# atonderski/future-object-detection

Hardware: AMD Instinct MI355X
Metric: frame-sequences/sec fwd+bwd, T=6 900x1600 (higher is better)
Workload: dtype bf16; 1 GPU; spatiotemporal ConditionalDETR (ResNet-50, 6 enc + 6 dec layers, 128 queries), T=6 frames 900x1600, batch 2/GPU, num_images K=5 (5 past frames live), random-init weights; step = forward (incl. Hungarian set loss, post-proc, AP bookkeeping) + backward + clip + AdamW; global_batch=2, frames=6, num_images=5, parallelism=dp1

## Files before the change

### future-object-detection_amd/csrc/api.cpp

```cpp
#include <stdarg.h>
#include <stdio.h>
#include <stdlib.h>
#include <string.h>

#include <mutex>

#include "../../include/fod.h"
#include "knobs.h"

static thread_local char g_err[512] = "";

void fod_set_error(const char* fmt, ...) {
  va_list ap;
  va_start(ap, fmt);
  vsnprintf(g_err, sizeof(g_err), fmt, ap);
  va_end(ap);
}

extern "C" size_t fod_last_error(char* buf, size_t cap) {
  const size_t n = strlen(g_err);
  if (buf && cap) {
    const size_t c = n < cap - 1 ? n : cap - 1;
    memcpy(buf, g_err, c);
    buf[c] = 0;
  }
  return n;
}

extern "C" int fod_abi_version(void) { return FOD_ABI_VERSION; }

extern "C" size_t fod_workspace_bytes(int kind) {
  switch (kind) {
    case FOD_WS_NT_SPLIT: return (size_t)FOD_NT_SPLIT_WS_FLOATS * sizeof(float);
    case FOD_WS_NT_SPLIT_TICKETS: return (size_t)FOD_NT_SPLIT_TICKETS * sizeof(unsigned);
    case FOD_WS_TN_PARTIALS: return FOD_TN_WS_BYTES;
    case FOD_WS_ATTN_SPLIT_PER_TILE: return (size_t)FOD_ATTN_SPLIT_WS_FLOATS_PER_TILE * sizeof(float);
    case FOD_WS_DET: return FOD_DET_WS_BYTES;
    case FOD_WS_TN_MULTI_DET: return FOD_TN_MULTI_DET_WS_BYTES;
    default: return 0;
  }
}

namespace {
struct KnobName {
  const char* name;
  int Knobs::*i;
  double Knobs::*d;
};
const KnobName KNOB_NAMES[] = {
    {"FOD_NT_SMALL", &Knobs::nt_small, nullptr},
    {"FOD_NT_NARROW", &Knobs::nt_narrow, nullptr},
    {"FOD_NT_SPLITK", &Knobs::nt_splitk, nullptr},
    {"FOD_NT_BIG", &Knobs::nt_big, nullptr},
    {"FOD_NT_BIG256", &Knobs::nt_big256, nullptr},
    {"FOD_NT_BIG_ILV", &Knobs::nt_big_ilv, nullptr},
    {"FOD_NT_BIG256_MINK", &Knobs::nt_big256_mink, nullptr},
    {"FOD_NT_BIG_MINK", &Knobs::nt_big_mink, nullptr},
    {"FOD_NT_BIG_MINN", &Knobs::nt_big_minn, nullptr},
    {"FOD_TN_SMALL", &Knobs::tn_small, nullptr},
    {"FOD_TN_BIG", &Knobs::tn_big, nullptr},
    {"FOD_TN_BIG_DENSE", &Knobs::tn_big_dense, nullptr},
    {"FOD_TN_BIG256", &Knobs::tn_big256, nullptr},
    {"FOD_TN_BIG_MIN", nullptr, &Knobs::tn_big_min},
    {"FOD_TN_BIG_SPLITS", &Knobs::tn_big_splits, nullptr},
    {"FOD_TN_WS", &Knobs::tn_ws, nullptr},
    {"FOD_TN_XCD", &Knobs::tn_xcd, nullptr},
    {"FOD_TN_ROWS", &Knobs::tn_rows, nullptr},
    {"FOD_ATTN_LDS", &Knobs::attn_lds, nullptr},
    {"FOD_ATTN_PF", &Knobs::attn_pf, nullptr},
    {"FOD_FP8_STAGE", &Knobs::fp8_stage, nullptr},
    {"FOD_LN_BWD_GROUPS", &Knobs::ln_bwd_groups, nullptr},
    {"FOD_BNK_VERSION", &Knobs::bnk_version, nullptr},
};

bool knob_parse(const KnobName& k, const char* text, Knobs& t) {
  char* end = nullptr;
  if (k.d) {
    const double v = strtod(text, &end);
    if (end == text || *end) return false;
    t.*k.d = v;
    return true;
  }
  if (Knobs{}.*k.i == Knobs::AUTO && !strcmp(text, "auto")) {
    t.*k.i = Knobs::AUTO;
    return true;
  }
  const long v = strtol(text, &end, 10);
  if (end == text || *end || v < 0 || v > 0x7FFFFFFF) return false;
  t.*k.i = (int)v;
  return true;
}

std::mutex g_knob_mutex;
Knobs& knob_table() {
  static Knobs table = [] {
    Knobs t;
    for (const KnobName& k : KNOB_NAMES)
      if (const char* text = getenv(k.name)) knob_parse(k, text, t);
    return t;
  }();
  return table;
}
const KnobName* knob_find(const char* name) {
  for (const KnobName& k : KNOB_NAMES)
    if (name && !strcmp(name, k.name)) return &k;
// ... 43 lines not shown
```

### future-object-detection_amd/csrc/common.h

```cpp
#pragma once
#include <hip/hip_runtime.h>
#include <stdint.h>

#include <mutex>

#include "../../include/fod.h"

typedef __attribute__((ext_vector_type(8))) __bf16 bf16x8_t;
typedef __attribute__((ext_vector_type(4))) __bf16 bf16x4_t;
typedef __attribute__((ext_vector_type(16))) float f32x16;
typedef __attribute__((ext_vector_type(4))) float f32x4;
typedef __attribute__((ext_vector_type(4))) short short4_t;

#define FOD_DEVINL __device__ __forceinline__

void fod_set_error(const char* fmt, ...);
#define FOD_REQUIRE(cond, ...)          \
  do {                                  \
    if (!(cond)) {                      \
      fod_set_error(__VA_ARGS__);       \
      return FOD_ERR_ARG;               \
    }                                   \
  } while (0)
#define FOD_LAUNCH_CHECK()                                              \
// ... 64 lines not shown
  for (int j = 0; j < 8; ++j) acc = __builtin_amdgcn_mfma_f32_32x32x2f32(a.v[j], b.v[j], acc, 0, 0, 0);
}

FOD_DEVINL void frag_load_contig(Frag<__bf16>& f, const __bf16* p) {
  f.v = *reinterpret_cast<const bf16x8_t*>(p);
}
FOD_DEVINL void frag_load_contig(Frag<float>& f, const float* p) {
  const f32x4 a = *reinterpret_cast<const f32x4*>(p);
  const f32x4 b = *reinterpret_cast<const f32x4*>(p + 4);
  f.v[0] = a[0]; f.v[1] = a[1]; f.v[2] = a[2]; f.v[3] = a[3];
  f.v[4] = b[0]; f.v[5] = b[1]; f.v[6] = b[2]; f.v[7] = b[3];
}
template <typename T>
FOD_DEVINL void frag_zero(Frag<T>& f) {
#pragma unroll
  for (int j = 0; j < 8; ++j) f.v[j] = (T)0.f;
}
template <typename T>
FOD_DEVINL void frag_from_acc(Frag<T>& f, const f32x16& acc, int s) {
#pragma unroll
  for (int j = 0; j < 8; ++j) f.v[j] = (T)acc[8 * s + j];
}
template <typename T>
FOD_DEVINL void frag_gather_accorder(Frag<T>& f, const T* base, long stride, int s, int h, int nrows) {
#pragma unroll
  for (int j = 0; j < 8; ++j) {
    const int r = 16 * s + 8 * (j >> 2) + 4 * h + (j & 3);
    f.v[j] = (r < nrows) ? base[(long)r * stride] : (T)0.f;
  }
}

FOD_DEVINL unsigned drop_mix(unsigned i, unsigned seed_lo, unsigned seed_hi) {
  unsigned h = (i ^ seed_lo) * 0x9E3779B1u + seed_hi;
  h ^= h >> 15;
  h *= 0x85EBCA77u;
  h ^= h >> 13;
  h *= 0xC2B2AE3Du;
  h ^= h >> 16;
  return h;
}

FOD_DEVINL unsigned long long mix64(unsigned long long x) {
  x = (x ^ (x >> 30)) * 0xBF58476D1CE4E5B9ull;
  x = (x ^ (x >> 27)) * 0x94D049BB133111EBull;
  return x ^ (x >> 31);
}
FOD_DEVINL unsigned long long effective_seed(unsigned long long seed, const unsigned long long* base_dev) {
  return base_dev ? mix64(seed + *base_dev) : seed;
}

FOD_DEVINL void store_sc1(float* p, float v) { __hip_atomic_store(p, v, __ATOMIC_RELAXED, __HIP_MEMORY_SCOPE_AGENT); }
FOD_DEVINL float load_sc1(const float* p) { return __hip_atomic_load(p, __ATOMIC_RELAXED, __HIP_MEMORY_SCOPE_AGENT); }
FOD_DEVINL void stores_done() { asm volatile("s_waitcnt vmcnt(0)" ::: "memory"); }

FOD_DEVINL int acc_row(int reg, int lane) { return (reg & 3) + 8 * (reg >> 2) + 4 * (lane >> 5); }

FOD_DEVINL float wave_sum(float v) {
#pragma unroll
  for (int o = 32; o > 0; o >>= 1) v += __shfl_xor(v, o);
  return v;
}
FOD_DEVINL float wave_max(float v) {
#pragma unroll
  for (int o = 32; o > 0; o >>= 1) v = fmaxf(v, __shfl_xor(v, o));
  return v;
}

static inline int ceil_div(long a, long b) { return (int)((a + b - 1) / b); }

struct LdsLimitOnce {
  std::once_flag once[64];
  int rc[64];
};
static inline int fod_lds_limit_once(LdsLimitOnce& st, const void* kernel, size_t bytes, const char* who) {
  int dev = 0;
  if (hipGetDevice(&dev) != hipSuccess || dev < 0 || dev >= 64) {
    fod_set_error("%s: no current device", who);
    return FOD_ERR_RUNTIME;
  }
  std::call_once(st.once[dev], [&] {
    st.rc[dev] = hipFuncSetAttribute(kernel, hipFuncAttributeMaxDynamicSharedMemorySize, (int)bytes) == hipSuccess ? 0 : 1;
  });
  if (st.rc[dev]) {
    fod_set_error("%s: cannot raise the dynamic LDS limit to %zu", who, bytes);
    return FOD_ERR_RUNTIME;
  }
  return FOD_OK;
}
```

### future-object-detection_amd/csrc/gemm_nt.hip

```cpp
#include <stdlib.h>

#include <type_traits>

#include "common.h"
#include "gemm_nt.h"
#include "gemm_tn.h"

namespace {

using namespace fodnt;

template <typename T, int MODE, int NT, bool UTAP>
FOD_DEVINL void gemm_nt_body(const NtParams& p) {
  constexpr int VEC = Elem<T>::VEC;
  constexpr int BK = ROW_BYTES / (int)sizeof(T);
  constexpr int BN = 64 * NT;
  constexpr int KSTEPS = BK / 16;
  constexpr int BROWS = BN / 32;
  extern __shared__ __attribute__((aligned(16))) unsigned char smem[];
  unsigned char* sA = smem;
  unsigned char* sB = smem + 2 * BM * ROW_BYTES;

  const int tid = threadIdx.x;
  const int lane = tid & 63;
  const int wave = tid >> 6;
  const int wm = wave >> 1, wn = wave & 1;
  FOD_STAMP(0);
  const int xcd = blockIdx.x & 7, slot = blockIdx.x >> 3;
  const int nt_i = slot % p.gx;
  const int mt_i = (slot / p.gx) * 8 + xcd;
  if (mt_i >= p.gy) return;
  const int n0 = nt_i * BN;
  const int m0 = mt_i * BM;
  const int cc = tid & 7;
  const int r0 = tid >> 3;

  constexpr unsigned OOB = 0xFFFFFFF0u;
  const auto rsA = __builtin_amdgcn_make_buffer_rsrc(const_cast<void*>(p.A), 0, p.a_bytes, 0x00020000);
  const auto rsB = __builtin_amdgcn_make_buffer_rsrc(const_cast<void*>(p.B), 0, p.b_bytes, 0x00020000);

  unsigned a_base[4];
  int a_h[4], a_w[4];
  int px_img = 0, px_h = 0, px_w = 0;
  if (MODE != MODE_DENSE) {
    const int mfirst = m0 + r0;
    const int hw = p.Hd * p.Wd;
    px_img = mfirst / hw;
    const int rem = mfirst - px_img * hw;
    px_h = rem / p.Wd;
    px_w = rem - px_h * p.Wd;
  }
#pragma unroll
  for (int i = 0; i < 4; ++i) {
    const int m = m0 + r0 + 32 * i;
    const bool valid = m < p.M;
    if (MODE == MODE_DENSE) {
      const int row = p.a_row_mod > 0 ? (m % p.a_row_mod) : m;
// ... 484 lines not shown
#pragma unroll
    for (int j = 0; j < 2; ++j)
#pragma unroll
      for (int r = 0; r < 16; ++r) acc[i][j][r] = 0.f;
  auto compute = [&](const Unit& f) {
#pragma unroll
    for (int ks = 0; ks < 2; ++ks)
#pragma unroll
      for (int i = 0; i < 2; ++i)
#pragma unroll
        for (int j = 0; j < 2; ++j) mma16(f.a[ks][i], f.b[ks][j], acc[i][j]);
  };
  Unit f0, f1;
  load_unit(ub, f0);
  load_unit(ub + 1, f1);
  FOD_STAMP(1);
  for (int u = ub; u < ue; u += 2) {
    compute(f0);
    load_unit(u + 2, f0);
    if (u + 1 < ue) compute(f1);
    load_unit(u + 3, f1);
  }

  FOD_STAMP(2);
#pragma unroll
  for (int i = 0; i < 2; ++i)
#pragma unroll
    for (int j = 0; j < 2; ++j)
#pragma unroll
      for (int r = 0; r < 16; ++r) sC[wave][i * 32 + acc_row(r, lane)][j * 32 + fr] = acc[i][j][r];
  __syncthreads();
  FOD_STAMP(3);
  const bool has_scale = p.scale != nullptr, has_mask = p.mask != nullptr;
  long c_base = bz * p.c_batch;
  int n_c = n;
  if (p.c_seg_cols > 0) {
    const int cseg = n0 / p.c_seg_cols;
    c_base += (long)cseg * p.c_seg_stride;
    n_c = n - cseg * p.c_seg_cols;
  }
  f32x4 vsum[4];
#pragma unroll
  for (int ps = 0; ps < 4; ++ps) {
    const int row = rq + 16 * ps;
    vsum[ps] = *reinterpret_cast<const f32x4*>(&sC[0][row][cq * 4]);
#pragma unroll
    for (int w = 1; w < 4; ++w) vsum[ps] += *reinterpret_cast<const f32x4*>(&sC[w][row][cq * 4]);
  }
  if (KS > 1) {
    __shared__ unsigned s_ticket;
    const long tile = (long)blockIdx.y * gridDim.x + blockIdx.x;
    float* mine = p.split_ws + (tile * KS + kz) * 4096;
#pragma unroll
    for (int ps = 0; ps < 4; ++ps)
#pragma unroll
      for (int e = 0; e < 4; ++e) store_sc1(mine + (rq + 16 * ps) * 64 + cq * 4 + e, vsum[ps][e]);
    stores_done();
    __syncthreads();
    if (tid == 0) s_ticket = atomicAdd(p.split_tickets + tile, 1u);
    __syncthreads();
    if (s_ticket != (unsigned)(KS - 1)) return;
    const float* all = p.split_ws + tile * KS * 4096;
#pragma unroll
    for (int ps = 0; ps < 4; ++ps) vsum[ps] = f32x4{0.f, 0.f, 0.f, 0.f};
    for (int z = 0; z < KS; ++z)
#pragma unroll
      for (int ps = 0; ps < 4; ++ps)
#pragma unroll
        for (int e = 0; e < 4; ++e) vsum[ps][e] += load_sc1(all + z * 4096 + (rq + 16 * ps) * 64 + cq * 4 + e);
    if (tid == 0) p.split_tickets[tile] = 0u;
  }
#pragma unroll
  for (int ps = 0; ps < 4; ++ps) {
    const int row = rq + 16 * ps;
    const int m = m0 + row;
    f32x4 v = vsum[ps];
    if (has_scale) v = v * sc;
    v += sh;
#pragma unroll
    for (int e = 0; e < 4; ++e) v[e] += (float)rres[ps][e];
    if (p.relu) {
#pragma unroll
      for (int e = 0; e < 4; ++e) v[e] = fmaxf(v[e], 0.f);
    }
    if (has_mask) {
#pragma unroll
      for (int e = 0; e < 4; ++e) v[e] = ((float)rmsk[ps][e] > 0.f) ? v[e] : 0.f;
    }
    if (m < p.M && n_ok) {
      if (p.c_is_f32) {
        *reinterpret_cast<f32x4*>(reinterpret_cast<float*>(p.C) + c_base + (long)m * p.ldc + n_c) = v;
      } else {
        *reinterpret_cast<bf16x4_t*>(reinterpret_cast<__bf16*>(p.C) + c_base + (long)m * p.ldc + n_c) =
            bf16x4_t{(__bf16)v[0], (__bf16)v[1], (__bf16)v[2], (__bf16)v[3]};
      }
    }
  }
  FOD_STAMP(4);
}

template <typename T, int MODE>
int launch_128(const NtParams& p, const NtRoute& r, hipStream_t stream) {
  NtParams q = p;
  q.gy = ceil_div(p.M, BM);
  const bool narrow = r.tile_n == 64;
  const dim3 block(256);
  constexpr int BK = ROW_BYTES / (int)sizeof(T);
  const bool utap = MODE != MODE_DENSE && MODE != MODE_STEM && p.Cs % BK == 0;
  q.gx = ceil_div(p.N, r.tile_n);
  const dim3 grid(q.gx * ((q.gy + 7) / 8 * 8));
  const size_t lds = 2 * (BM + r.tile_n) * ROW_BYTES;
#define FOD_NT_LAUNCH(KERNEL_NT1, KERNEL_NT2)                                        \
  do {                                                                               \
    if (narrow) hipLaunchKernelGGL((KERNEL_NT1), grid, block, lds, stream, q);       \
    else hipLaunchKernelGGL((KERNEL_NT2), grid, block, lds, stream, q);              \
  } while (0)
  if constexpr (MODE == MODE_DENSE) {
    FOD_NT_LAUNCH((gemm_nt_kernel<T, 1>), (gemm_nt_kernel<T, 2>));
  } else if constexpr (MODE == MODE_STEM) {
    FOD_NT_LAUNCH((conv_stem_fwd_kernel<T, 1>), (conv_stem_fwd_kernel<T, 2>));
  } else if constexpr (MODE == MODE_CONV) {
    if (utap) FOD_NT_LAUNCH((conv2d_fwd_kernel<T, 1, true>), (conv2d_fwd_kernel<T, 2, true>));
// ... 160 lines not shown
  FOD_REQUIRE(out && (dtype == FOD_BF16 || dtype == FOD_F32), "gemm_nt_route: bad args");
  NtParams p{};
  if (int rc = dense_params(p, dtype, nullptr, lda, a_row_mod, nullptr, ldb, nullptr, ldc, M, N, K, epi)) return rc;
  *out = route(MODE_DENSE, dtype, p, fod_knobs());
  return FOD_OK;
}

extern "C" int fod_gemm_nt_grouped(int dtype, const void* A, long lda, int a_seg_len, long a_seg_stride,
                                   const void* B, long ldb, void* C, long ldc, int c_seg_cols, long c_seg_stride,
                                   int M, int N, int K, const fod_epilogue* epi, int res_nseg, long res_seg_stride,
                                   hipStream_t stream) {
  FOD_REQUIRE(dtype == FOD_BF16, "gemm_nt_grouped: bf16 only (dtype %d)", dtype);
  FOD_REQUIRE(A && B && C, "gemm_nt_grouped: null operand");
  FOD_REQUIRE(M > 0 && N > 0 && K > 0, "gemm_nt_grouped: empty problem %d %d %d", M, N, K);
  FOD_REQUIRE(K % 8 == 0 && lda % 8 == 0 && ldb % 8 == 0, "gemm_nt_grouped: K=%d lda=%ld ldb=%ld must be multiples of 8",
              K, lda, ldb);
  FOD_REQUIRE(((uintptr_t)A % 16) == 0 && ((uintptr_t)B % 16) == 0, "gemm_nt_grouped: operands must be 16-byte aligned");
  FOD_REQUIRE(a_seg_len >= 0 && c_seg_cols >= 0, "gemm_nt_grouped: negative segment size");
  FOD_REQUIRE(a_seg_len == 0 || (a_seg_len % 32 == 0 && K % a_seg_len == 0 && a_seg_stride % 8 == 0),
              "gemm_nt_grouped: A segments of %d (stride %ld) must be multiples of 32 dividing K=%d", a_seg_len,
              a_seg_stride, K);
  FOD_REQUIRE(c_seg_cols == 0 || (c_seg_cols % 64 == 0 && c_seg_stride % 4 == 0),
              "gemm_nt_grouped: C segments of %d columns (stride %ld) must be multiples of 64 / 4", c_seg_cols,
              c_seg_stride);
  NtParams p{};
  p.A = A; p.B = B; p.C = C;
  p.lda = lda; p.ldb = ldb; p.ldc = ldc;
  p.M = M; p.N = N; p.K = K;
  p.a_seg_len = a_seg_len; p.a_seg_stride = a_seg_stride;
  p.c_seg_cols = c_seg_cols; p.c_seg_stride = c_seg_stride;
  fill_epilogue(p, epi);
  decide_vec_epilogue(p);
  FOD_REQUIRE(p.vec_epi, "gemm_nt_grouped: N, ldc and the epilogue operands must be 4-element / 16-byte aligned");
  FOD_REQUIRE(res_nseg >= 0 && (res_nseg == 0 || (p.res && c_seg_cols > 0 && res_seg_stride % 4 == 0 &&
                                                  res_nseg <= ceil_div(N, c_seg_cols))),
              "gemm_nt_grouped: per-segment residual (%d blocks) needs a residual, C segments and a 4-element block stride", res_nseg);
  p.res_nseg = res_nseg;
  p.res_seg_stride = res_seg_stride;
  FOD_REQUIRE(!p.res || ((long)(res_nseg > 1 ? res_nseg - 1 : 0) * res_seg_stride +
                         (long)(p.res_row_mod > 0 ? p.res_row_mod : M) * p.ldr + N) * 2 < 0x7FFFFFF0L,
              "gemm_nt_grouped: residual larger than 2 GiB");
  FOD_REQUIRE(!p.mask || ((long)M * p.ldmask + N) * 2 < 0x7FFFFFF0L, "gemm_nt_grouped: mask larger than 2 GiB");
  const long nseg = a_seg_len > 0 ? K / a_seg_len : 1;
  const long seg_k = a_seg_len > 0 ? a_seg_len : K;
  const long ab = ((nseg - 1) * a_seg_stride + (long)(M - 1) * lda + seg_k) * 2, bb = ((long)(N - 1) * ldb + K) * 2;
  FOD_REQUIRE(ab < 0xFFFFFFF0L - 16 && bb < 0xFFFFFFF0L - 16, "gemm_nt_grouped: operand larger than 4 GiB");
  p.a_bytes = (unsigned)ab;
  p.b_bytes = (unsigned)bb;
  hipLaunchKernelGGL(gemm_nt_small_kernel, dim3(ceil_div(N, 64), ceil_div(M, 64)), dim3(256), 0, stream, p);
  FOD_LAUNCH_CHECK();
  return FOD_OK;
}

extern "C" int fod_gemm_nt_batched(int dtype, int batches, const void* A, long lda, long a_batch, const void* B, long ldb,
                                   long b_batch, void* C, long ldc, long c_batch, int M, int N, int K,
                                   const fod_epilogue* epi, long shift_batch, long residual_batch, long mask_batch,
                                   hipStream_t stream) {
  FOD_REQUIRE(dtype == FOD_BF16, "gemm_nt_batched: bf16 only (dtype %d)", dtype);
  FOD_REQUIRE(A && B && C && batches > 0, "gemm_nt_batched: null operand / no batch");
  FOD_REQUIRE(M > 0 && N > 0 && K > 0, "gemm_nt_batched: empty problem %d %d %d", M, N, K);
  FOD_REQUIRE(K % 8 == 0 && lda % 8 == 0 && ldb % 8 == 0, "gemm_nt_batched: K=%d lda=%ld ldb=%ld must be multiples of 8",
              K, lda, ldb);
  FOD_REQUIRE(a_batch % 8 == 0 && b_batch % 8 == 0 && c_batch % 8 == 0 && shift_batch % 4 == 0 && residual_batch % 8 == 0 &&
                  mask_batch % 8 == 0,
              "gemm_nt_batched: batch strides must keep every operand 16-byte aligned");
  FOD_REQUIRE(((uintptr_t)A % 16) == 0 && ((uintptr_t)B % 16) == 0, "gemm_nt_batched: operands must be 16-byte aligned");
  NtParams p{};
  p.A = A; p.B = B; p.C = C;
  p.lda = lda; p.ldb = ldb; p.ldc = ldc;
  p.M = M; p.N = N; p.K = K;
  fill_epilogue(p, epi);
  p.split_ws = nullptr; p.split_tickets = nullptr;
  decide_vec_epilogue(p);
  FOD_REQUIRE(p.vec_epi, "gemm_nt_batched: N, ldc and the epilogue operands must be 4-element / 16-byte aligned");
  FOD_REQUIRE(!p.res || p.res_row_mod == 0, "gemm_nt_batched: no periodic residual");
  FOD_REQUIRE(!p.res || ((long)M * p.ldr + N) * 2 < 0x7FFFFFF0L, "gemm_nt_batched: residual larger than 2 GiB");
  FOD_REQUIRE(!p.mask || ((long)M * p.ldmask + N) * 2 < 0x7FFFFFF0L, "gemm_nt_batched: mask larger than 2 GiB");
  const long ab = ((long)(M - 1) * lda + K) * 2, bb = ((long)(N - 1) * ldb + K) * 2;
  FOD_REQUIRE(ab < 0xFFFFFFF0L - 16 && bb < 0xFFFFFFF0L - 16, "gemm_nt_batched: operand larger than 4 GiB");
  p.a_bytes = (unsigned)ab;
  p.b_bytes = (unsigned)bb;
  const long gy = (long)ceil_div(M, 64) * batches;
  FOD_REQUIRE(gy <= 65535, "gemm_nt_batched: %ld row tiles x batches exceed the grid", gy);
  p.batches = batches;
  p.a_batch = a_batch; p.b_batch = b_batch; p.c_batch = c_batch;
  p.shift_batch = shift_batch; p.res_batch = residual_batch; p.mask_batch = mask_batch;
  hipLaunchKernelGGL(gemm_nt_small_kernel, dim3(ceil_div(N, 64), (unsigned)gy), dim3(256), 0, stream, p);
  FOD_LAUNCH_CHECK();
  return FOD_OK;
}

namespace {
int conv_params(NtParams& p, int dtype, bool dgrad, const void* src, const void* w, void* dst, const fod_conv_geom* g,
                const fod_epilogue* epi) {
  const int vec = dtype == FOD_BF16 ? 8 : 4;
  FOD_REQUIRE(g->stride == 1 || g->stride == 2, "conv: stride %d unsupported", g->stride);
  const int Ho = (g->H + 2 * g->pad - g->kh) / g->stride + 1;
  const int Wo = (g->W + 2 * g->pad - g->kw) / g->stride + 1;
  FOD_REQUIRE(Ho == g->Ho && Wo == g->Wo, "conv: geometry mismatch Ho=%d/%d Wo=%d/%d", g->Ho, Ho, g->Wo, Wo);
  FOD_REQUIRE(g->Cin % vec == 0 && g->Cout % vec == 0, "conv: channels %d/%d must be multiples of %d",
              g->Cin, g->Cout, vec);
  FOD_REQUIRE(((uintptr_t)src % 16) == 0 && ((uintptr_t)w % 16) == 0, "conv: operands must be 16-byte aligned");
  p.A = src; p.B = w; p.C = dst;
  p.kh = g->kh; p.kw = g->kw; p.stride = g->stride; p.pad = g->pad;
  if (!dgrad) {
    p.Hs = g->H; p.Ws = g->W; p.Cs = g->Cin;
// ... 125 lines not shown
```

### future-object-detection_amd/csrc/knobs.h

```cpp
#pragma once

struct Knobs {
  static constexpr int AUTO = -1;
  int nt_small = 1;
  int nt_narrow = AUTO;
  int nt_splitk = AUTO;
  int nt_big = 1;
  int nt_big256 = 1;
  int nt_big_ilv = AUTO;
  int nt_big256_mink = 128;
  int nt_big_mink = 1536;
  int nt_big_minn = 256;
  int tn_small = 1;
  int tn_big = 1;
  int tn_big_dense = 0;
  int tn_big256 = 0;
  double tn_big_min = 2.0e9;
  int tn_big_splits = 0;
  int tn_ws = 1;
  int tn_xcd = 1;
  int tn_rows = 0;
  int attn_lds = 8;
  int attn_pf = 1;
  int fp8_stage = 1;
  int ln_bwd_groups = 4;
  int bnk_version = 4;
};

Knobs fod_knobs();
```

### future-object-detection_amd/future_od/native/lib.py

```python
import contextlib
import ctypes as C
import os

from . import abi
from .abi import FodError
from ..switches import SW

LIB_PATH = os.path.normpath(os.path.join(os.path.dirname(os.path.abspath(__file__)), "..", "..", "lib", "libfod_hip.so"))

globals().update({name[4:].replace("ROUTE_", "", 1): value for name, value in abi.CONSTANTS.items()})

_i, _l, _f, _p = C.c_int, C.c_long, C.c_float, C.c_void_p


def _struct(name, c_name):
    return type(name, (C.Structure,), {"_fields_": [(field, abi.CTYPE[kind]) for field, kind in abi.STRUCTS[c_name]]})


Epilogue = _struct("Epilogue", "fod_epilogue")
ConvGeom = _struct("ConvGeom", "fod_conv_geom")
AttnShape = _struct("AttnShape", "fod_attn_shape")
PermuteJob = _struct("PermuteJob", "fod_permute_job")
TnJob = _struct("TnJob", "fod_tn_job")
NtRoute = _struct("NtRoute", "fod_nt_route")
TnRoute = _struct("TnRoute", "fod_tn_route")
AttnRoute = _struct("AttnRoute", "fod_attn_kernels")

EXPORTS = sorted(abi.PROTOTYPES)
SIGNATURES = {name: [abi.CTYPE[kind] for kind in args] for name, args in abi.served(abi.PROTOTYPES).items()}
EXT_EXPORTS = sorted(abi.EXT_PROTOTYPES)
EXT_SIGNATURES = {name: [abi.CTYPE[kind] for kind in args] for name, args in abi.served(abi.EXT_PROTOTYPES).items()}


def _typed(lib, name):
    ret, args = abi.PROTOTYPES[name] if name in abi.PROTOTYPES else abi.EXT_PROTOTYPES[name]
    fn = getattr(lib, name)
    fn.restype, fn.argtypes = abi.CTYPE[ret], [abi.CTYPE[kind] for kind in args]
    return fn


def _load():
    if not os.path.isfile(LIB_PATH):
        raise FodError(
            f"{LIB_PATH} not found: build it with `python -c 'import __graft_entry__ as g; g.build()'` "
            "(or future-object-detection_amd/build.sh). There is no fallback path.")
    import torch
    lib = C.CDLL(LIB_PATH)
    built = _typed(lib, "fod_abi_version")()
    if built != abi.CONSTANTS["FOD_ABI_VERSION"]:
        raise FodError(f"libfod_hip.so ABI {built} != header ABI {abi.CONSTANTS['FOD_ABI_VERSION']}: rebuild")
    for name in EXPORTS + EXT_EXPORTS:
        if not hasattr(lib, name):
            raise FodError(f"libfod_hip.so does not export {name}: rebuild")
        _typed(lib, name)
    return lib


LIB = _load()


def last_error():
    buf = C.create_string_buffer(512)
    LIB.fod_last_error(buf, 512)
    return buf.value.decode("utf-8", "replace")


def knob(name):
    buf = C.create_string_buffer(32)
    if LIB.fod_knob_get(name.encode(), buf, 32) != 0:
        raise FodError(f"fod_knob_get failed: {last_error()}")
    return buf.value.decode()


def set_knob(name, value):
    if LIB.fod_knob_set(name.encode(), None if value is None else str(value).encode()) != 0:
        raise FodError(f"fod_knob_set failed: {last_error()}")


@contextlib.contextmanager
def knobs(**values):
    old = {name: knob(name) for name in values}
    try:
        for name, value in values.items():
            set_knob(name, value)
        yield
    finally:
        for name, value in old.items():
            set_knob(name, value)


def _load_fast():
    import importlib.util
    path = os.path.join(os.path.dirname(LIB_PATH), "_fodfast.so")
    if not os.path.isfile(path) or not SW.FOD_FASTCALL:
        return {}
    spec = importlib.util.spec_from_file_location("_fodfast", path)
    mod = importlib.util.module_from_spec(spec)
    spec.loader.exec_module(mod)
    return {name: getattr(mod, name) for name in SIGNATURES if hasattr(mod, name)}


FAST = _load_fast()
_ENTRY = {name: FAST.get(name, getattr(LIB, name)) for name in SIGNATURES}
_ENTRY.update({name: getattr(LIB, name) for name in EXT_SIGNATURES})


def _plain_call(name, *args):
    rc = _ENTRY[name](*args)
    if rc != 0:
        raise FodError(f"{name} failed ({rc}): {last_error()}")


class Profiler:

    def __init__(self):
        self.enabled = False
        self.records = []
        self.pending_work = 0.0

    def start(self):
        self.enabled = True
        self.records = []

    def stop(self):
        self.enabled = False

    def summary(self):
# ... 29 lines not shown
```

### future-object-detection_amd/future_od/native/ops.py

```python
import ctypes as C
import math

import torch

from . import abi, capture
from . import lib as L
from .lib import F32, BF16, AttnShape, ConvGeom, Epilogue
from .. import switches
from ..switches import SW


def call(name, *args, **kw):
    return L.call(name, *args, **kw)

_DT = {torch.float32: F32, torch.bfloat16: BF16}


def dt(t):
    try:
        return _DT[t.dtype]
    except KeyError:
        raise L.FodError(f"unsupported activation dtype {t.dtype}") from None


# ... 7 lines not shown


class _Addr(int):

    def __new__(cls, struct):
        self = super().__new__(cls, C.addressof(struct))
        self.keep = struct
        return self


def ptr(t):
    if t is None:
        return None
    return t.data_ptr()


def _chk(t, name, dtype=None):
    if not t.is_cuda:
        raise L.FodError(f"{name}: expected a device tensor (the HIP path has no CPU fallback)")
    if not t.is_contiguous():
        raise L.FodError(f"{name}: expected a contiguous tensor, got strides {t.stride()} for {tuple(t.shape)}")
    if dtype is not None and t.dtype != dtype:
        raise L.FodError(f"{name}: expected {dtype}, got {t.dtype}")
    return t


_WS = {}


def _workspace(kind, device, captured=None):
    if captured is None:
        captured = torch.cuda.is_current_stream_capturing()
    key = (kind, device.index, "graph" if captured else stream())
    hit = _WS.get(key)
    if hit is None:
        nbytes = L.LIB.fod_workspace_bytes(kind)
        hit = torch.zeros(nbytes // 4, dtype=torch.int32, device=device)
        _WS[key] = hit
    if captured:
        capture.hold_or_ask("scratch", hit)
    return hit


def preallocate_graph_workspaces(device):
    device = torch.device(device)
    kinds = (L.WS_NT_SPLIT, L.WS_NT_SPLIT_TICKETS, L.WS_TN_PARTIALS)
    if SW.FOD_DETERMINISTIC:
        kinds += (L.WS_DET, L.WS_TN_MULTI_DET)
    for kind in kinds:
        _workspace(kind, device, captured=True)
    tiles = max((hit[2] for key, hit in _ATTN_SPLIT.items() if key[0] == device.index), default=0)
    if tiles:
        _attn_split_workspace(device, tiles, captured=True)


def set_deterministic(flag):
    switches.set("FOD_DETERMINISTIC", bool(flag))


def is_deterministic():
    return SW.FOD_DETERMINISTIC


def det_workspace(device, kind=L.WS_DET):
    ws = _workspace(kind, device)
    return ws.data_ptr(), ws.numel() * 4


_DET_TWINS = abi.det_twins(abi.PROTOTYPES)


def call_twin(name, device, *args, **kw):
    if not SW.FOD_DETERMINISTIC:
        return call(name, *args, stream(), **kw)
    scratch = det_workspace(device) if _DET_TWINS[name] else ()
    return call(name + "_det", *args, *scratch, stream(), **kw)


def nt_wants_split_ws(M, N, K):
    return K >= 1024 and ((M + 63) // 64) * ((N + 63) // 64) <= 64


def tn_may_use_partials_ws(M):
    return M >= 8192


def _epi(scale=None, shift=None, residual=None, ld_residual=0, residual_row_mod=0, relu_mask=None,
         ld_mask=0, relu=False, out_f32=False, split_for=None):
    want_split = split_for is not None and nt_wants_split_ws(*split_for[1:])
    if (scale is None and shift is None and residual is None and relu_mask is None and not relu and not out_f32
            and not want_split):
        return None
    ws = tk = None
    if want_split:
        ws, tk = _workspace(L.WS_NT_SPLIT, split_for[0]), _workspace(L.WS_NT_SPLIT_TICKETS, split_for[0])
    e = Epilogue(ptr(scale), ptr(shift), ptr(residual), ld_residual, residual_row_mod,
                 ptr(relu_mask), ld_mask, int(relu), int(out_f32), ptr(ws), ptr(tk))
    return _Addr(e)


def tn_workspace(device):
    ws = _workspace(L.WS_TN_PARTIALS, device)
    return ws.data_ptr(), ws.numel() * 4


_THERE = 16


def gemm_nt_route(M, N, K, dtype=torch.bfloat16):
    e, r = Epilogue(), L.NtRoute()
    if dtype == torch.bfloat16 and nt_wants_split_ws(M, N, K):
        e.split_ws = e.split_tickets = _THERE
    call("fod_gemm_nt_route", _DT[dtype], K, 0, K, N, M, N, K, C.addressof(e), C.addressof(r))
    return r


def _tn_ws_bytes(M):
    return L.LIB.fod_workspace_bytes(L.WS_TN_PARTIALS) if tn_may_use_partials_ws(M) or SW.FOD_DETERMINISTIC else 0


def gemm_tn_route(M, N1, K2, dtype=torch.bfloat16, row_scale=False, colsum=False):
    r = L.TnRoute()
    call("fod_gemm_tn_route", _DT[dtype], M, N1, K2, N1, K2, K2, int(row_scale), int(colsum), int(SW.FOD_DETERMINISTIC),
         _tn_ws_bytes(M), C.addressof(r))
    return r


def conv2d_route(which, geom, dtype=torch.bfloat16):
    r = L.TnRoute() if which == L.CONV_WGRAD else L.NtRoute()
    call("fod_conv2d_route", which, _DT[dtype], C.addressof(geom), None, int(SW.FOD_DETERMINISTIC),
         _tn_ws_bytes(geom.Nimg * geom.Ho * geom.Wo), C.addressof(r))
    return r


def gemm_nt(a, b, *, a_row_mod=0, m_rows=None, scale=None, shift=None, residual=None,
            residual_row_mod=0, relu=False, relu_mask=None, out_f32=False, out=None):
    _chk(a, "a"); _chk(b, "b", a.dtype)
    K = a.shape[-1]
    N = b.shape[0]
    assert b.shape[1] == K, (a.shape, b.shape)
    a_rows = a.numel() // K
    M = m_rows if m_rows is not None else a_rows
    if a_row_mod:
        assert a_row_mod <= a_rows
    else:
        assert M <= a_rows
    for v, n in ((scale, "scale"), (shift, "shift")):
        if v is not None:
            _chk(v, n, torch.float32); assert v.numel() == N
    if residual is not None:
        _chk(residual, "residual", a.dtype)
        assert residual.shape[-1] == N
        rr = residual.numel() // N
        assert (residual_row_mod and residual_row_mod <= rr) or (not residual_row_mod and rr >= M)
    if relu_mask is not None:
        _chk(relu_mask, "relu_mask", a.dtype)
        assert relu_mask.numel() == M * N
    if out is None:
        out = torch.empty((M, N), dtype=torch.float32 if out_f32 else a.dtype, device=a.device)
    else:
        _chk(out, "out"); assert out.numel() == M * N
    call("fod_gemm_nt", dt(a), ptr(a), K, a_row_mod, ptr(b), K, ptr(out), N, M, N, K,
         _epi(scale, shift, residual, N, residual_row_mod, relu_mask, N, relu, out_f32,
              split_for=(a.device, M, N, K) if a.dtype == torch.bfloat16 else None), stream(),
         work=2.0 * M * N * K)
    return out


def gemm_nt_batched(a, b, *, b_cols=False, shift=None, residual=None, relu=False, relu_mask=None):
    _chk(a, "a", torch.bfloat16); _chk(b, "b", torch.bfloat16)
    P, M, K = a.shape
    if b_cols:
        N = b.shape[0]
        assert b.dim() == 2 and b.shape[1] == P * K, (a.shape, b.shape)
        ldb, b_batch = P * K, K
    else:
        N = b.numel() // (P * K)
        assert b.shape[-1] == K and N * P * K == b.numel(), (a.shape, b.shape)
        ldb, b_batch = K, N * K
    if shift is not None:
        _chk(shift, "shift", torch.float32); assert shift.numel() == P * N
    for v, n in ((residual, "residual"), (relu_mask, "relu_mask")):
        if v is not None:
            _chk(v, n, torch.bfloat16); assert v.numel() == P * M * N
    out = torch.empty((P, M, N), dtype=a.dtype, device=a.device)
    call("fod_gemm_nt_batched", dt(a), P, ptr(a), K, M * K, ptr(b), ldb, b_batch, ptr(out), N, M * N, M, N, K,
         _epi(None, shift, residual, N, 0, relu_mask, N, relu, False), N, M * N, M * N, stream(),
         work=2.0 * P * M * N * K, tag="fod_gemm_nt")
    return out


def gemm_tn_acc(g, x, dw, row_scale=None, colsum=None, zeroed=False):
    _chk(g, "g"); _chk(x, "x", g.dtype); _chk(dw, "dw", torch.float32)
    N1, K2 = g.shape[-1], x.shape[-1]
    M = g.numel() // N1
    assert x.numel() // K2 == M and dw.numel() == N1 * K2, (g.shape, x.shape, dw.shape)
    if row_scale is not None:
        _chk(row_scale, "row_scale", torch.float32); assert row_scale.numel() == N1
    if colsum is not None:
        _chk(colsum, "colsum", torch.float32); assert colsum.numel() == N1
    ws, ws_bytes = tn_workspace(g.device) if _tn_ws_bytes(M) else (None, 0)
    call_twin("fod_gemm_tn_acc", g.device, dt(g), ptr(g), N1, ptr(x), K2, ptr(dw), K2, M, N1, K2, ptr(row_scale),
              ptr(colsum), 0 if zeroed else 1, ws, ws_bytes, work=2.0 * M * N1 * K2, tag="fod_gemm_tn_acc")
    return dw


def group_linear_fwd(x, wcat, bcat, P, relu=False, residual=None, res_row_mod=0):
    _chk(x, "x", torch.bfloat16); _chk(wcat, "wcat", torch.bfloat16)
    K = x.shape[-1]
    rows = x.numel() // K
    N = wcat.shape[0]
    D = N // P
    assert wcat.shape[1] == K and N == P * D and D % 64 == 0, (x.shape, wcat.shape, P)
    if bcat is not None:
        _chk(bcat, "bcat", torch.float32); assert bcat.numel() == N
    y = torch.empty((P, rows, D), dtype=x.dtype, device=x.device)
    nseg, seg_stride = 0, 0
    if residual is not None:
        _chk(residual, "residual", x.dtype)
        nseg, R = residual.shape[0], residual.shape[1]
        assert residual.dim() == 3 and residual.shape[2] == D and nseg <= P
        assert (res_row_mod and res_row_mod <= R) or (not res_row_mod and R >= rows)
        seg_stride = R * D
    call("fod_gemm_nt_grouped", dt(x), ptr(x), K, 0, 0, ptr(wcat), K, ptr(y), D, D, rows * D, rows, N, K,
         _epi(None, bcat, residual, D, res_row_mod, None, N, relu, False), nseg, seg_stride, stream(),
         work=2.0 * rows * N * K, tag="fod_gemm_nt")
    return y


def group_linear_dgrad(g, wcat_t, P):
    _chk(g, "g", torch.bfloat16); _chk(wcat_t, "wcat_t", torch.bfloat16)
    _, rows, D = g.shape
    K = wcat_t.shape[0]
    assert g.shape[0] == P and wcat_t.shape[1] == P * D and D % 32 == 0
    dx = torch.empty((rows, K), dtype=g.dtype, device=g.device)
    call("fod_gemm_nt_grouped", dt(g), ptr(g), D, D, rows * D, ptr(wcat_t), P * D, ptr(dx), K, 0, 0, rows, K, P * D,
         None, 0, 0, stream(), work=2.0 * rows * K * P * D, tag="fod_gemm_nt")
    return dx


def group_linear_wgrad(g, x, dw, db, zeroed=False):
    _chk(g, "g", torch.bfloat16); _chk(x, "x", torch.bfloat16); _chk(dw, "dw", torch.float32)
    P, rows, D = g.shape
    K = x.shape[-1]
    assert x.numel() // K == rows and dw.numel() == P * D * K and D % 64 == 0
    if db is not None:
        _chk(db, "db", torch.float32); assert db.numel() == P * D
    call("fod_gemm_tn_grouped", dt(g), ptr(g), D, D, rows * D, ptr(x), K, ptr(dw), K, rows, P * D, K, ptr(db),
         0 if zeroed else 1, stream(), work=2.0 * rows * P * D * K, tag="fod_gemm_tn_acc")
    return dw


def colsum_acc(g, out, group_rows=0):
    _chk(g, "g"); _chk(out, "out", torch.float32)
    N = g.shape[-1]
    M = g.numel() // N
    groups = 1 if group_rows <= 0 else (M + group_rows - 1) // group_rows
    assert out.numel() == groups * N, (g.shape, out.shape, group_rows)
    call_twin("fod_colsum_acc", g.device, dt(g), ptr(g), N, M, N, group_rows, ptr(out))
    return out


def conv_geom(x_shape, cout, k, stride, pad):
    n, h, w, cin = x_shape
    ho = (h + 2 * pad - k) // stride + 1
    wo = (w + 2 * pad - k) // stride + 1
    return ConvGeom(n, h, w, cin, ho, wo, cout, k, k, stride, pad)


def _conv_flops(g, cin=None):
    return 2.0 * g.Nimg * g.Ho * g.Wo * g.Cout * g.kh * g.kw * (g.Cin if cin is None else cin)


def conv2d_fwd(x, w, geom, *, scale=None, shift=None, residual=None, relu=False, work_cin=None, out=None):
    _chk(x, "x"); _chk(w, "w", x.dtype)
    assert tuple(x.shape) == (geom.Nimg, geom.H, geom.W, geom.Cin), (x.shape, geom.H, geom.W, geom.Cin)
    assert w.numel() == geom.Cout * geom.kh * geom.kw * geom.Cin
    if out is None:
        y = torch.empty((geom.Nimg, geom.Ho, geom.Wo, geom.Cout), dtype=x.dtype, device=x.device)
    else:
        y = _chk(out, "out", x.dtype)
        assert tuple(y.shape) == (geom.Nimg, geom.Ho, geom.Wo, geom.Cout), (y.shape,)
    for v in (scale, shift):
        if v is not None:
            _chk(v, "scale/shift", torch.float32); assert v.numel() == geom.Cout
    if residual is not None:
        _chk(residual, "residual", x.dtype); assert residual.shape == y.shape
    call("fod_conv2d_fwd", dt(x), ptr(x), ptr(w), ptr(y), _Addr(geom),
# ... 770 lines not shown
```

### include/fod.h

```cpp
#ifndef FOD_H_
#define FOD_H_

#include <stddef.h>
#include <stdint.h>

#ifdef __cplusplus
extern "C" {
#endif

typedef struct ihipStream_t* fod_stream_t;

enum { FOD_F32 = 0, FOD_BF16 = 1 };
enum { FOD_OK = 0, FOD_ERR_ARG = 1, FOD_ERR_LAUNCH = 2, FOD_ERR_RUNTIME = 3 };

size_t fod_last_error(char* buf, size_t cap);
int fod_abi_version(void);
#define FOD_ABI_VERSION 12

int fod_knob_set(const char* name, const char* value);
int fod_knob_get(const char* name, char* out, size_t out_bytes);

enum { FOD_ROUTE_NT_SMALL = 0,
       FOD_ROUTE_NT_128 = 1,
       FOD_ROUTE_NT_BIG = 2 };
typedef struct fod_nt_route {
  int kernel;
  int tile_n;
  int stages;
  int interleave;
  int ksplit;
  int wants_split_ws;
} fod_nt_route;
enum { FOD_ROUTE_TN_SMALL = 0,
       FOD_ROUTE_TN_128 = 1,
       FOD_ROUTE_TN_BIG = 2 };
typedef struct fod_tn_route {
  int kernel;
  int bi, bj;
  int nsplit;
  int m_per_split;
  int xcd_order;
  int uses_partials_ws;
} fod_tn_route;

typedef struct fod_epilogue {
  const float* scale;
  const float* shift;
  const void* residual;
  long ld_residual;
  int residual_row_mod;
  const void* relu_mask;
  long ld_mask;
  int relu;
  int out_f32;
  void* split_ws;
  void* split_tickets;
} fod_epilogue;
#define FOD_NT_SPLIT_WS_FLOATS (64 * 8 * 4096)
#define FOD_NT_SPLIT_TICKETS 64
#define FOD_TN_WS_BYTES ((size_t)64 << 20)
enum { FOD_WS_NT_SPLIT = 0, FOD_WS_NT_SPLIT_TICKETS = 1, FOD_WS_TN_PARTIALS = 2, FOD_WS_ATTN_SPLIT_PER_TILE = 3,
       FOD_WS_DET = 4, FOD_WS_TN_MULTI_DET = 5 };
size_t fod_workspace_bytes(int kind);
#define FOD_DET_WS_BYTES ((size_t)16 << 20)
#define FOD_TN_MULTI_DET_WS_BYTES ((size_t)128 << 20)
#define FOD_TN_DET_MAX_SPLITS 4

int fod_gemm_nt(int dtype, const void* A, long lda, int a_row_mod, const void* B, long ldb, void* C,
                long ldc, int M, int N, int K, const fod_epilogue* epi, fod_stream_t stream);

// ... 293 lines not shown
```

### include/fod_ext.h

```cpp
#ifndef FOD_EXT_H_
#define FOD_EXT_H_

#include "fod.h"

#ifdef __cplusplus
extern "C" {
#endif

int fod_multi_ema(const long* pairs, const long* numel, const int* blk_tensor, const int* blk_chunk, int nblocks,
                  const long long* updates_dev, float decay, int warmup, fod_stream_t stream);
int fod_multi_swap(const long* pairs, const long* numel, const int* blk_tensor, const int* blk_chunk, int nblocks,
                   fod_stream_t stream);
int fod_multi_accum(const long* pairs, const long* numel, const int* blk_tensor, const int* blk_chunk, int nblocks,
                    int mode, float scale, fod_stream_t stream);
int fod_clip_crop_resize_photo(const unsigned char* src, float* dst, int B, int L, int C, int H0, int W0, int H, int W,
                               long src_stride_b, long src_stride_l, const int* plans, const float* mean,
                               const float* std, const float* photo, fod_stream_t stream);

#ifdef __cplusplus
}
#endif
#endif
```

Baseline: 108.9 frame-sequences/s.

## Add split-K deep GEMM path for small-tile, long-K NT GEMMs and grouped dgrad

Adds a new entry point that launches the small NT GEMM kernel with a split-K grid chosen by a planner. It applies when the output has few 64x64 tiles but a long K dimension, such as grouped linear dgrad and some plain gemm_nt calls, so that more CUs get work. It also vectorises the split-K partial store and reduction with 16-byte sc1 loads and stores. The cost is extra scratch traffic, a ticket-based reduction, and new workspace management for graph capture.

New measurement: 109.8 frame-sequences/s, median of 6. No clear change (+0.8%).

```diff
diff --git a/future-object-detection_amd/csrc/api.cpp b/future-object-detection_amd/csrc/api.cpp
--- a/future-object-detection_amd/csrc/api.cpp
+++ b/future-object-detection_amd/csrc/api.cpp
@@ -51,6 +51,7 @@
     {"FOD_NT_SMALL", &Knobs::nt_small, nullptr},
     {"FOD_NT_NARROW", &Knobs::nt_narrow, nullptr},
     {"FOD_NT_SPLITK", &Knobs::nt_splitk, nullptr},
+    {"FOD_NT_DEEP", &Knobs::nt_deep, nullptr},
     {"FOD_NT_BIG", &Knobs::nt_big, nullptr},
     {"FOD_NT_BIG256", &Knobs::nt_big256, nullptr},
     {"FOD_NT_BIG_ILV", &Knobs::nt_big_ilv, nullptr},
diff --git a/future-object-detection_amd/csrc/common.h b/future-object-detection_amd/csrc/common.h
--- a/future-object-detection_amd/csrc/common.h
+++ b/future-object-detection_amd/csrc/common.h
@@ -140,6 +140,25 @@
 FOD_DEVINL void store_sc1(float* p, float v) { __hip_atomic_store(p, v, __ATOMIC_RELAXED, __HIP_MEMORY_SCOPE_AGENT); }
 FOD_DEVINL float load_sc1(const float* p) { return __hip_atomic_load(p, __ATOMIC_RELAXED, __HIP_MEMORY_SCOPE_AGENT); }
 FOD_DEVINL void stores_done() { asm volatile("s_waitcnt vmcnt(0)" ::: "memory"); }
+FOD_DEVINL void store_sc1_16(float* p, f32x4 v) {
+  asm volatile("global_store_dwordx4 %0, %1, off sc1\n\ts_nop 1" ::"v"(p), "v"(v) : "memory");
+}
+FOD_DEVINL void load_sc1_16x8(f32x4 (&a)[4], f32x4 (&b)[4], const float* pa, const float* pb, int stride) {
+  asm volatile(
+      "global_load_dwordx4 %0, %8, off sc1\n\t"
+      "global_load_dwordx4 %1, %9, off sc1\n\t"
+      "global_load_dwordx4 %2, %10, off sc1\n\t"
+      "global_load_dwordx4 %3, %11, off sc1\n\t"
+      "global_load_dwordx4 %4, %12, off sc1\n\t"
+      "global_load_dwordx4 %5, %13, off sc1\n\t"
+      "global_load_dwordx4 %6, %14, off sc1\n\t"
+      "global_load_dwordx4 %7, %15, off sc1\n\t"
+      "s_waitcnt vmcnt(0)"
+      : "=&v"(a[0]), "=&v"(a[1]), "=&v"(a[2]), "=&v"(a[3]), "=&v"(b[0]), "=&v"(b[1]), "=&v"(b[2]), "=&v"(b[3])
+      : "v"(pa), "v"(pa + stride), "v"(pa + 2 * stride), "v"(pa + 3 * stride), "v"(pb), "v"(pb + stride),
+        "v"(pb + 2 * stride), "v"(pb + 3 * stride)
+      : "memory");
+}
 
 FOD_DEVINL int acc_row(int reg, int lane) { return (reg & 3) + 8 * (reg >> 2) + 4 * (lane >> 5); }
 
diff --git a/future-object-detection_amd/csrc/gemm_nt.hip b/future-object-detection_amd/csrc/gemm_nt.hip
--- a/future-object-detection_amd/csrc/gemm_nt.hip
+++ b/future-object-detection_amd/csrc/gemm_nt.hip
@@ -3,6 +3,7 @@
 #include <type_traits>
 
 #include "common.h"
+#include "../../include/fod_ext.h"
 #include "gemm_nt.h"
 #include "gemm_tn.h"
 
@@ -593,9 +594,7 @@
     const long tile = (long)blockIdx.y * gridDim.x + blockIdx.x;
     float* mine = p.split_ws + (tile * KS + kz) * 4096;
 #pragma unroll
-    for (int ps = 0; ps < 4; ++ps)
-#pragma unroll
-      for (int e = 0; e < 4; ++e) store_sc1(mine + (rq + 16 * ps) * 64 + cq * 4 + e, vsum[ps][e]);
+    for (int ps = 0; ps < 4; ++ps) store_sc1_16(mine + (rq + 16 * ps) * 64 + cq * 4, vsum[ps]);
     stores_done();
     __syncthreads();
     if (tid == 0) s_ticket = atomicAdd(p.split_tickets + tile, 1u);
@@ -604,11 +603,18 @@
     const float* all = p.split_ws + tile * KS * 4096;
 #pragma unroll
     for (int ps = 0; ps < 4; ++ps) vsum[ps] = f32x4{0.f, 0.f, 0.f, 0.f};
-    for (int z = 0; z < KS; ++z)
-#pragma unroll
-      for (int ps = 0; ps < 4; ++ps)
-#pragma unroll
-        for (int e = 0; e < 4; ++e) vsum[ps][e] += load_sc1(all + z * 4096 + (rq + 16 * ps) * 64 + cq * 4 + e);
+    for (int z = 0; z < KS; z += 2) {
+      f32x4 pa[4], pb[4];
+      const bool two = z + 1 < KS;
+      const float* mine_r = all + (rq * 64 + cq * 4);
+      load_sc1_16x8(pa, pb, mine_r + z * 4096, mine_r + (two ? z + 1 : z) * 4096, 16 * 64);
+#pragma unroll
+      for (int ps = 0; ps < 4; ++ps) vsum[ps] += pa[ps];
+      if (two) {
+#pragma unroll
+        for (int ps = 0; ps < 4; ++ps) vsum[ps] += pb[ps];
+      }
+    }
     if (tid == 0) p.split_tickets[tile] = 0u;
   }
 #pragma unroll
@@ -875,6 +881,78 @@
   return FOD_OK;
 }
 
+namespace {
+int deep_ksplit(int M, int N, int K, int a_seg_len, const Knobs& kn) {
+  if (kn.nt_deep == 0 || !kn.nt_small) return 1;
+  const long tiles = (long)ceil_div(M, 64) * ceil_div(N, 64);
+  if (tiles > 256) return 1;
+  if (kn.nt_deep >= 2) return kn.nt_deep < 8 ? kn.nt_deep : 8;
+  if (K < 1024 || (a_seg_len == 0 && tiles <= 64)) return 1;
+  if (tiles > 64) return 4;
+  int ks = (int)(512 / tiles);
+  if (ks > 8) ks = 8;
+  if (ks > K / 256) ks = K / 256;
+  return ks;
+}
+}
+
+extern "C" int fod_gemm_nt_deep_plan(int M, int N, int K, int a_seg_len, int* ksplit, size_t* ws_bytes,
+                                     size_t* ticket_bytes) {
+  FOD_REQUIRE(ksplit && ws_bytes && ticket_bytes, "gemm_nt_deep_plan: null result");
+  FOD_REQUIRE(M > 0 && N > 0 && K > 0 && a_seg_len >= 0, "gemm_nt_deep_plan: bad problem %d %d %d (segments of %d)", M, N, K,
+              a_seg_len);
+  const int ks = deep_ksplit(M, N, K, a_seg_len, fod_knobs());
+  const size_t tiles = (size_t)ceil_div(M, 64) * ceil_div(N, 64);
+  *ksplit = ks;
+  *ws_bytes = ks > 1 ? tiles * ks * 4096 * sizeof(float) : 0;
+  *ticket_bytes = ks > 1 ? tiles * sizeof(unsigned) : 0;
+  return FOD_OK;
+}
+
+extern "C" int fod_gemm_nt_deep(int dtype, const void* A, long lda, int a_seg_len, long a_seg_stride, const void* B,
+                                long ldb, void* C, long ldc, int M, int N, int K, const fod_epilogue* epi, void* ws,
+                                size_t ws_bytes, void* tickets, size_t ticket_bytes, hipStream_t stream) {
+  FOD_REQUIRE(dtype == FOD_BF16, "gemm_nt_deep: bf16 only (dtype %d)", dtype);
+  FOD_REQUIRE(A && B && C && ws && tickets, "gemm_nt_deep: null operand or scratch");
+  FOD_REQUIRE(M > 0 && N > 0 && K > 0, "gemm_nt_deep: empty problem %d %d %d", M, N, K);
+  FOD_REQUIRE(K % 8 == 0 && lda % 8 == 0 && ldb % 8 == 0, "gemm_nt_deep: K=%d lda=%ld ldb=%ld must be multiples of 8", K, lda,
+              ldb);
+  FOD_REQUIRE(((uintptr_t)A % 16) == 0 && ((uintptr_t)B % 16) == 0 && ((uintptr_t)ws % 16) == 0 &&
+                  ((uintptr_t)tickets % 4) == 0,
+              "gemm_nt_deep: operands and scratch must be 16-byte aligned (tickets: 4)");
+  FOD_REQUIRE(a_seg_len >= 0 && (a_seg_len == 0 || (a_seg_len % 32 == 0 && K % a_seg_len == 0 && a_seg_stride % 8 == 0)),
+              "gemm_nt_deep: A segments of %d (stride %ld) must be multiples of 32 dividing K=%d", a_seg_len, a_seg_stride, K);
+  NtParams p{};
+  p.A = A; p.B = B; p.C = C;
+  p.lda = lda; p.ldb = ldb; p.ldc = ldc;
+  p.M = M; p.N = N; p.K = K;
+  p.a_seg_len = a_seg_len; p.a_seg_stride = a_seg_len > 0 ? a_seg_stride : 0;
+  fill_epilogue(p, epi);
+  decide_vec_epilogue(p);
+  FOD_REQUIRE(p.vec_epi, "gemm_nt_deep: N, ldc and the epilogue operands must be 4-element / 16-byte aligned");
+  FOD_REQUIRE(!p.res || ((long)(p.res_row_mod > 0 ? p.res_row_mod : M) * p.ldr + N) * 2 < 0x7FFFFFF0L,
+              "gemm_nt_deep: residual larger than 2 GiB");
+  FOD_REQUIRE(!p.mask || ((long)M * p.ldmask + N) * 2 < 0x7FFFFFF0L, "gemm_nt_deep: mask larger than 2 GiB");
+  const long nseg = a_seg_len > 0 ? K / a_seg_len : 1;
+  const long seg_k = a_seg_len > 0 ? a_seg_len : K;
+  const long ab = ((nseg - 1) * p.a_seg_stride + (long)(M - 1) * lda + seg_k) * 2, bb = ((long)(N - 1) * ldb + K) * 2;
+  FOD_REQUIRE(ab < 0xFFFFFFF0L - 16 && bb < 0xFFFFFFF0L - 16, "gemm_nt_deep: operand larger than 4 GiB");
+  p.a_bytes = (unsigned)ab;
+  p.b_bytes = (unsigned)bb;
+  const int ks = deep_ksplit(M, N, K, a_seg_len, fod_knobs());
+  FOD_REQUIRE(ks > 1, "gemm_nt_deep: the plan answers 1 split for %d x %d x %d: not this entry point's problem", M, N, K);
+  const size_t tiles = (size_t)ceil_div(M, 64) * ceil_div(N, 64);
+  FOD_REQUIRE(ws_bytes >= tiles * ks * 4096 * sizeof(float) && ticket_bytes >= tiles * sizeof(unsigned),
+              "gemm_nt_deep: scratch of %zu + %zu bytes is smaller than the plan's %zu + %zu", ws_bytes, ticket_bytes,
+              tiles * ks * 4096 * sizeof(float), tiles * sizeof(unsigned));
+  p.ksplit = ks;
+  p.split_ws = reinterpret_cast<float*>(ws);
+  p.split_tickets = reinterpret_cast<unsigned*>(tickets);
+  hipLaunchKernelGGL(gemm_nt_small_kernel, dim3(ceil_div(N, 64), ceil_div(M, 64), ks), dim3(256), 0, stream, p);
+  FOD_LAUNCH_CHECK();
+  return FOD_OK;
+}
+
 extern "C" int fod_gemm_nt_batched(int dtype, int batches, const void* A, long lda, long a_batch, const void* B, long ldb,
                                    long b_batch, void* C, long ldc, long c_batch, int M, int N, int K,
                                    const fod_epilogue* epi, long shift_batch, long residual_batch, long mask_batch,
diff --git a/future-object-detection_amd/csrc/knobs.h b/future-object-detection_amd/csrc/knobs.h
--- a/future-object-detection_amd/csrc/knobs.h
+++ b/future-object-detection_amd/csrc/knobs.h
@@ -5,6 +5,7 @@
   int nt_small = 1;
   int nt_narrow = AUTO;
   int nt_splitk = AUTO;
+  int nt_deep = AUTO;
   int nt_big = 1;
   int nt_big256 = 1;
   int nt_big_ilv = AUTO;
diff --git a/future-object-detection_amd/future_od/native/lib.py b/future-object-detection_amd/future_od/native/lib.py
--- a/future-object-detection_amd/future_od/native/lib.py
+++ b/future-object-detection_amd/future_od/native/lib.py
@@ -72,7 +72,11 @@
     return buf.value.decode()
 
 
+KNOB_EPOCH = [0]
+
+
 def set_knob(name, value):
+    KNOB_EPOCH[0] += 1
     if LIB.fod_knob_set(name.encode(), None if value is None else str(value).encode()) != 0:
         raise FodError(f"fod_knob_set failed: {last_error()}")
 
diff --git a/future-object-detection_amd/future_od/native/ops.py b/future-object-detection_amd/future_od/native/ops.py
--- a/future-object-detection_amd/future_od/native/ops.py
+++ b/future-object-detection_amd/future_od/native/ops.py
@@ -83,6 +83,9 @@
     tiles = max((hit[2] for key, hit in _ATTN_SPLIT.items() if key[0] == device.index), default=0)
     if tiles:
         _attn_split_workspace(device, tiles, captured=True)
+    deep = [hit for key, hit in _NT_DEEP.items() if key[0] == device.index]
+    if deep:
+        _nt_deep_workspace(device, max(h[2] for h in deep), max(h[3] for h in deep), captured=True)
 
 
 def set_deterministic(flag):
@@ -162,6 +165,51 @@
     call("fod_conv2d_route", which, _DT[dtype], C.addressof(geom), None, int(SW.FOD_DETERMINISTIC),
          _tn_ws_bytes(geom.Nimg * geom.Ho * geom.Wo), C.addressof(r))
     return r
+
+
+_DEEP_PLANS = {}
+_DEEP_PLANS_EPOCH = [0]
+
+
+def nt_deep_plan(M, N, K, a_seg_len=0):
+    if _DEEP_PLANS_EPOCH[0] != L.KNOB_EPOCH[0]:
+        _DEEP_PLANS.clear()
+        _DEEP_PLANS_EPOCH[0] = L.KNOB_EPOCH[0]
+    key = (M, N, K, a_seg_len)
+    hit = _DEEP_PLANS.get(key)
+    if hit is None:
+        ks, wb, tb = C.c_int(), C.c_size_t(), C.c_size_t()
+        L._plain_call("fod_gemm_nt_deep_plan", M, N, K, a_seg_len, C.addressof(ks), C.addressof(wb), C.addressof(tb))
+        hit = _DEEP_PLANS[key] = (ks.value, wb.value, tb.value)
+    return hit
+
+
+_NT_DEEP = {}
+
+
+def _nt_deep_workspace(device, ws_floats, tiles, captured=None):
+    if captured is None:
+        captured = torch.cuda.is_current_stream_capturing()
+    key = (device.index, "graph" if captured else stream())
+    hit = _NT_DEEP.get(key)
+    if hit is None or hit[2] < ws_floats or hit[3] < tiles:
+        ws_floats, tiles = max(ws_floats, hit[2] if hit else 0), max(tiles, hit[3] if hit else 0, 256)
+        hit = (torch.empty(ws_floats, dtype=torch.float32, device=device),
+               torch.zeros(tiles, dtype=torch.int32, device=device), ws_floats, tiles)
+        _NT_DEEP[key] = hit
+    if captured:
+        capture.hold_or_ask("deep GEMM split scratch", hit)
+    return hit
+
+
+def _gemm_nt_deep(plan, a, lda, a_seg_len, a_seg_stride, b, ldb, out, ldc, M, N, K, epi, work):
+    ws, tk, ws_floats, tiles = _nt_deep_workspace(a.device, plan[1] // 4, plan[2] // 4)
+    call("fod_gemm_nt_deep", dt(a), ptr(a), lda, a_seg_len, a_seg_stride, ptr(b), ldb, ptr(out), ldc, M, N, K, epi,
+         ptr(ws), ws_floats * 4, ptr(tk), tiles * 4, stream(), work=work, tag="fod_gemm_nt")
+
+
+def _aligned16(*tensors):
+    return all(t is None or t.data_ptr() % 16 == 0 for t in tensors)
 
 
 def gemm_nt(a, b, *, a_row_mod=0, m_rows=None, scale=None, shift=None, residual=None,
@@ -191,6 +239,12 @@
         out = torch.empty((M, N), dtype=torch.float32 if out_f32 else a.dtype, device=a.device)
     else:
         _chk(out, "out"); assert out.numel() == M * N
+    if a.dtype == torch.bfloat16 and not a_row_mod:
+        plan = nt_deep_plan(M, N, K)
+        if plan[0] > 1 and N % 4 == 0 and _aligned16(out, scale, shift, residual, relu_mask):
+            _gemm_nt_deep(plan, a, K, 0, 0, b, K, out, N, M, N, K,
+                          _epi(scale, shift, residual, N, residual_row_mod, relu_mask, N, relu, out_f32), 2.0 * M * N * K)
+            return out
     call("fod_gemm_nt", dt(a), ptr(a), K, a_row_mod, ptr(b), K, ptr(out), N, M, N, K,
          _epi(scale, shift, residual, N, residual_row_mod, relu_mask, N, relu, out_f32,
               split_for=(a.device, M, N, K) if a.dtype == torch.bfloat16 else None), stream(),
@@ -265,6 +319,10 @@
     K = wcat_t.shape[0]
     assert g.shape[0] == P and wcat_t.shape[1] == P * D and D % 32 == 0
     dx = torch.empty((rows, K), dtype=g.dtype, device=g.device)
+    plan = nt_deep_plan(rows, K, P * D, D)
+    if plan[0] > 1:
+        _gemm_nt_deep(plan, g, D, D, rows * D, wcat_t, P * D, dx, K, rows, K, P * D, None, 2.0 * rows * K * P * D)
+        return dx
     call("fod_gemm_nt_grouped", dt(g), ptr(g), D, D, rows * D, ptr(wcat_t), P * D, ptr(dx), K, 0, 0, rows, K, P * D,
          None, 0, 0, stream(), work=2.0 * rows * K * P * D, tag="fod_gemm_nt")
     return dx
diff --git a/include/fod.h b/include/fod.h
--- a/include/fod.h
+++ b/include/fod.h
@@ -15,7 +15,7 @@
 
 size_t fod_last_error(char* buf, size_t cap);
 int fod_abi_version(void);
-#define FOD_ABI_VERSION 12
+#define FOD_ABI_VERSION 13
 
 int fod_knob_set(const char* name, const char* value);
 int fod_knob_get(const char* name, char* out, size_t out_bytes);
diff --git a/include/fod_ext.h b/include/fod_ext.h
--- a/include/fod_ext.h
+++ b/include/fod_ext.h
@@ -17,6 +17,11 @@
                                long src_stride_b, long src_stride_l, const int* plans, const float* mean,
                                const float* std, const float* photo, fod_stream_t stream);
 
+int fod_gemm_nt_deep_plan(int M, int N, int K, int a_seg_len, int* ksplit, size_t* ws_bytes, size_t* ticket_bytes);
+int fod_gemm_nt_deep(int dtype, const void* A, long lda, int a_seg_len, long a_seg_stride, const void* B, long ldb,
+                     void* C, long ldc, int M, int N, int K, const fod_epilogue* epi, void* ws, size_t ws_bytes,
+                     void* tickets, size_t ticket_bytes, fod_stream_t stream);
+
 #ifdef __cplusplus
 }
 #endif
```
